# kyutai-labs/pocket-tts

Measured on AMD Instinct MI355X. Metric: audio-seconds/sec (xRT), 100M en model, whole job over all GPUs, higher is better.
Workload: dtype f32

## Files before the change

### pocket_tts_amd/csrc/ptts.hip

```cpp
#include "ptts_host.h"
#include "ptts_flow.h"
#include "ptts_bf16.h"
#include "ptts_lm.h"

#include <algorithm>
#include <array>
#include <cmath>
#include <cstdio>
#include <cstring>

static thread_local std::string g_err;
int fail(int code, const std::string &msg) {
  g_err = msg;
  return code;
}
static thread_local std::string g_launch_err;
bool launch_err_pending() { return !g_launch_err.empty(); }
int take_launch_err() {
  std::string m;
  m.swap(g_launch_err);
  return fail(-4, m);
}
void note_launch_err(const std::string &msg) { if (g_launch_err.empty()) g_launch_err = msg; }

// ... 251 lines not shown
  launch_gemm(st, a, PRE_LNFOLD);
  AttnArgs at;
  at.Q = c.q; at.Kc = c.Kc; at.Vc = c.Vc; at.offset = c.offset; at.H = c.H; at.Tq = c.Tq; at.QB = c.QB;
  at.cap = c.cap; at.ring = c.ring; at.ctx = c.ctx; at.splits = c.splits; at.part = c.part; at.Y = c.ao; at.YF = DF; at.h16 = 0;
  at.pre = c.pre; at.layer = c.layer; at.qlen = c.qlen;
  const int BH = (c.M / c.Tq) * c.H;
  at.nseq = BH / c.H;
  SITE(s3.c_str());
  launch_attention(st, at, BH, c.cascade, -1, c.kv_keys * c.H * 64 * 4 * 2 + 8.0 * c.M * c.D,
                   4.0 * c.kv_keys * c.H * 64 * std::min(c.Tq, 16));
  SITE(s4.c_str());
  a = mk_gemm(T.out, c.ao, DF, c.MT, c.M);
  a.epi = EPI_RES; a.R = c.x_in; a.RF = DF; a.Y = c.x; a.YF = DF; a.ls = T.ls1;
  launch_gemm(st, a, PRE_NONE);
  SITE(s6.c_str());
  a = mk_gemm(T.ff1, c.x, DF, c.MT, c.M);
  a.epi = EPI_STORE; a.act = ACT_GELU; a.Y = c.ff; a.YF = c.FF / 16;
  launch_gemm(st, a, PRE_LNFOLD);
  SITE(s7.c_str());
  a = mk_gemm(T.ff2, c.ff, c.FF / 16, c.MT, c.M);
  a.epi = EPI_RES; a.R = c.x; a.RF = DF; a.Y = c.x_out; a.YF = DF; a.Ydstride = c.out_ds; a.par = c.par; a.ls = T.ls2;
  launch_gemm(st, a, PRE_NONE);
  SITE("");
}

extern "C" int ptts_abi_version(void) { return PTTS_ABI_VERSION; }
extern "C" const char *ptts_last_error(void) { return g_err.c_str(); }

static int seanet_check(const ptts_config &c) {
  if (c.d_model < 64 || c.num_heads < 1 || c.num_layers < 1 || c.m_dim < 64 || c.m_heads < 1 || c.m_layers < 1 || c.ldim < 16 ||
      c.flow_dim < 16 || c.flow_depth < 1 || c.ff_dim < 16 || c.m_ff < 16 || c.n_filters < 1 || c.compress < 1 ||
      c.kernel_size < 1 || c.res_kernel_size < 1 || c.last_kernel_size < 1 || c.ratios[0] < 1 || c.ratios[1] < 1 || c.ratios[2] < 1)
    return fail(-4, "model dimensions must be positive");
  if (c.d_model % 64 || c.d_model / c.num_heads != 64 || c.d_model % c.num_heads) return fail(-4, "FlowLM head dim must be 64");
  if (c.m_dim % c.m_heads || c.m_dim / c.m_heads != 64) return fail(-4, "Mimi head dim must be 64");
  if (c.d_model > 1024 || c.m_dim > 1024 || c.flow_dim > 1024) return fail(-4, "LayerNorm width > 1024 unsupported");
  if (c.ldim % 16 || c.flow_dim % 16 || c.ff_dim % 16 || c.m_ff % 16) return fail(-4, "dims must be multiples of 16");
  if (c.upsample_stride != 16) return fail(-4, "upsample stride must be 16 (one row tile per frame)");
  if ((c.n_filters / c.compress) % 16) return fail(-4, "n_filters/compress must be a multiple of 16");
  return 0;
}

static int build_engine(ptts_engine *e, const ptts_tensor *tensors, int32_t n);
static int build_fp8_codec(ptts_engine *e);
static int sync_host_tables(ptts_engine *e);

static int init_engine_options(ptts_engine *e, int device) {
  e->device = device;
  e->tuner = new Tuner();
  hipDeviceProp_t prop;
  HIPCHK(hipGetDeviceProperties(&prop, device));
  e->n_cus = std::max(1, prop.multiProcessorCount);
  if (const char *v = getenv("PTTS_FLOW_CLUSTER")) e->opt_flow_cluster = atoi(v) != 0;
  if (const char *v = getenv("PTTS_LM_CLUSTER")) e->opt_lm_cluster = atoi(v) != 0;
  if (const char *v = getenv("PTTS_K_ROTATE")) e->opt_k_rotate = atoi(v) != 0;
  if (const char *v = getenv("PTTS_FUSE_RES")) e->opt_fuse_res = atoi(v) != 0;
  if (const char *v = getenv("PTTS_SHARE_PREFIX")) e->opt_share_prefix = atoi(v) != 0;
  if (const char *v = getenv("PTTS_SINGLE_STORE")) e->opt_single_store = atoi(v) != 0;
  if (const char *v = getenv("PTTS_FUSE_PCM")) e->opt_fuse_pcm = atoi(v) != 0;
  if (const char *v = getenv("PTTS_CASCADE")) e->opt_cascade = atoi(v);
  if (const char *v = getenv("PTTS_FLOW_MAX_CUS")) e->opt_flow_max_cus = std::max(8, atoi(v));
  e->opt_flow_max_cus = std::min(e->opt_flow_max_cus, e->n_cus);
  if (const char *v = getenv("PTTS_CODEC_LDS_TARGET")) e->opt_codec_lds_target = std::max(0, std::min(atoi(v), 64 * 1024));
  return 0;
}

extern "C" int ptts_create(const ptts_config *cfg, const ptts_tensor *tensors, int32_t n, int32_t device,
                           ptts_engine **out) {
  return ptts_create_ex(cfg, tensors, n, device, 0, out);
}

extern "C" int ptts_create_ex(const ptts_config *cfg, const ptts_tensor *tensors, int32_t n, int32_t device,
                              int32_t quant_flags, ptts_engine **out) {
  if (!cfg || !tensors || !out) return fail(-1, "null argument");
  if (quant_flags & ~(PTTS_QUANT_ATTENTION | PTTS_QUANT_FFN | PTTS_CODEC_BF16 | PTTS_CODEC_FP8 | PTTS_LM_BF16 | PTTS_CODEC_SPLIT)) return fail(-1, "unknown quantisation group");
  if ((quant_flags & PTTS_CODEC_BF16) && (quant_flags & PTTS_CODEC_FP8)) return fail(-1, "PTTS_CODEC_BF16 and PTTS_CODEC_FP8 are exclusive");
  if ((quant_flags & PTTS_CODEC_SPLIT) && (quant_flags & (PTTS_CODEC_BF16 | PTTS_CODEC_FP8))) return fail(-1, "PTTS_CODEC_SPLIT and the bf16 / fp8 codec are exclusive");
  if ((quant_flags & PTTS_LM_BF16) && (quant_flags & (PTTS_QUANT_ATTENTION | PTTS_QUANT_FFN))) return fail(-1, "PTTS_LM_BF16 and the int8 groups are exclusive");
  CHK(seanet_check(*cfg));
  HIPCHK(hipSetDevice(device));
  ptts_engine *e = new ptts_engine();
  e->cfg = *cfg;
  e->quant_flags = quant_flags;
  int rc = init_engine_options(e, device);
  if (rc == 0) rc = build_engine(e, tensors, n);
  if (rc < 0) {
    const std::string msg = g_err;
    ptts_destroy(e);
    return fail(rc, msg);
  }
  *out = e;
  return 0;
}

static int build_engine(ptts_engine *e, const ptts_tensor *tensors, int32_t n) {
  HIPCHK(hipStreamCreateWithFlags(&e->stream, hipStreamNonBlocking));
  AllocScope alloc_scope(e->stream);
  HIPCHK(hipEventCreate(&e->ev0));
  HIPCHK(hipEventCreate(&e->ev1));
  for (int i = 0; i < n; ++i) e->tmap[tensors[i].name] = &tensors[i];
  const ptts_config &c = e->cfg;
  const int D = c.d_model, FD = c.flow_dim;
  std::string p = "flow_lm.";
  CHK(copy_vec(e, p + "bos_emb", c.ldim, &e->bos));
  CHK(make_freq(e, &e->freq_lm, c.max_period));
  CHK(pack_lin(e, &e->in_linear, {{p + "input_linear.weight", "", D}}, c.ldim, 1));
// ... 867 lines not shown
  if ((int64_t)out.size() + 1 > capacity) return fail(-1, "profile buffer too small");
  memcpy(h_out, out.c_str(), out.size() + 1);
  return (int64_t)out.size();
}


static bool flow_cluster_ok(const ptts_engine *e, const ptts_lm_state *s) {
  const ptts_config &c = e->cfg;
  const int FDF = c.flow_dim / 16, LF = c.ldim / 16;
  if (!e->opt_flow_cluster || c.flow_depth > FLOW_MAX_DEPTH || FDF > 64 || LF > FDF) return false;
  const int kpw = cdiv(std::max(FDF, LF), FLOW_WORKERS);
  if (kpw != 1 && kpw != 2 && kpw != 4) return false;
  if (!e->input_proj.bias || !e->fin.bias) return false;
  for (auto &r : e->res) if (!r.l0.bias || !r.l2.bias) return false;
  return FDF <= std::min(e->opt_flow_max_cus, e->n_cus);
}
static int ensure_flow(ptts_engine *e, ptts_lm_state *s, int steps, hipStream_t st) {
  if (steps <= s->flow_steps) return 0;
  if (s->n_graphs > 0)
    return fail(-1, "lsd_decode_steps grows beyond what this state's captured graphs were built for: destroy the graphs first "
                    "(they hold the old AdaLN / exchange buffers)");
  const ptts_config &c = e->cfg;
  const int FDF = c.flow_dim / 16;
  static const int rt_env = [] { const char *v = getenv("PTTS_FLOW_RT"); return v ? atoi(v) : 1; }();
  s->flow_rt = (rt_env == 2 && s->MT >= 2) ? 2 : 1;
  s->flow_ng = cdiv(s->MT, s->flow_rt);
  HIPCHK(hipStreamSynchronize(st));
  HIPCHK(hipStreamSynchronize(e->stream));
  AllocScope alloc_scope(st);
  hipFree(s->mod); hipFree(s->fexch); hipFree(s->fflags);
  s->mod = nullptr; s->fexch = nullptr; s->fflags = nullptr;
  const size_t rt = (size_t)s->MT * 256;
  const int nph = steps * (2 * c.flow_depth + 2);
  CHK(dallocT(nullptr, &s->mod, (size_t)steps * rt * e->adaln.NT));
  CHK(dallocT(nullptr, &s->fexch, (size_t)s->flow_ng * nph * s->flow_rt * FDF * 256));
  CHK(dallocT(nullptr, &s->fflags, (size_t)s->flow_ng * nph * FDF));
  HIPCHK(hipStreamSynchronize(st));
  s->flow_steps = steps;
  return 0;
}

template <int RT, bool ROWLSD>
static void launch_flow_rt(hipStream_t st, const FlowArgs &fa, int kpw) {
  const dim3 grid(fa.NCL * fa.FDF), block(FLOW_THREADS);
  switch (kpw) {
    case 1: flow_cluster_kernel<RT, 1, ROWLSD><<<grid, block, 0, st>>>(fa); break;
    case 2: flow_cluster_kernel<RT, 2, ROWLSD><<<grid, block, 0, st>>>(fa); break;
    default: flow_cluster_kernel<RT, 4, ROWLSD><<<grid, block, 0, st>>>(fa); break;
  }
}

static int flow_steps_of(const ptts_lm_state *s, int lsd_steps) { return std::max(lsd_steps, s->lsd_cap); }

static void launch_flow_cluster(hipStream_t st, ptts_engine *e, ptts_lm_state *s, int lsd_steps, float *d_latent_out) {
  const ptts_config &c = e->cfg;
  const int FDF = c.flow_dim / 16, LF = c.ldim / 16;
  FlowArgs fa;
  memset(&fa, 0, sizeof fa);
  fa.MT = s->MT; fa.M = s->B; fa.NG = s->flow_ng; fa.NCL = std::max(1, std::min(s->flow_ng, std::min(e->opt_flow_max_cus, e->n_cus) / FDF)); fa.FDF = FDF; fa.LF = LF; fa.AF = e->adaln.NT;
  const bool rowlsd = s->lsd_cap > 0;
  fa.depth = c.flow_depth; fa.steps = rowlsd ? flow_steps_of(s, lsd_steps) : lsd_steps; fa.ldim = c.ldim;
  fa.w_in = e->input_proj.w; fa.b_in = e->input_proj.bias;
  for (int r = 0; r < c.flow_depth; ++r) {
    fa.w_l0[r] = e->res[r].l0.w; fa.b_l0[r] = e->res[r].l0.bias;
    fa.w_l2[r] = e->res[r].l2.w; fa.b_l2[r] = e->res[r].l2.bias;
    fa.ln_w[r] = e->res[r].ln_w; fa.ln_b[r] = e->res[r].ln_b;
  }
  fa.w_fin = e->fin.w; fa.b_fin = e->fin.bias;
  fa.mod = s->mod; fa.mod_step = (long)s->MT * 256 * e->adaln.NT;
  fa.latfm = s->latfm;
  fa.lat = s->lat; fa.lat_out1 = s->lat_prev; fa.lat_out2 = d_latent_out;
  fa.inv_steps = 1.0f / (float)lsd_steps;
  fa.exch = s->fexch; fa.flags = s->fflags; fa.ctr = s->rng_ctr; fa.err = s->ferr;
  fa.row_n = rowlsd ? s->lsd_n : nullptr; fa.row_ndef = lsd_steps;
  const double wbytes = 4.0 * 256 * ((double)FDF * LF + 2.0 * c.flow_depth * FDF * FDF + (double)LF * FDF);
  const double flops = 2.0 * s->B * 256.0 * ((double)FDF * LF + 2.0 * c.flow_depth * FDF * FDF + (double)LF * FDF) * lsd_steps;
  ProfScope ps(st, std::string(rowlsd ? "flow_cluster_rowlsd@" : "flow_cluster@") + std::to_string((long)fa.NCL * FDF * FLOW_THREADS),
               lsd_steps * (wbytes + 4.0 * s->B * 16.0 * e->adaln.NT), flops);
  const int kpw = cdiv(std::max(FDF, LF), FLOW_WORKERS);
  s->coop_wgs = std::max(s->coop_wgs, fa.NCL * FDF);
  if (rowlsd) {
    if (s->flow_rt == 2) launch_flow_rt<2, true>(st, fa, kpw);
    else launch_flow_rt<1, true>(st, fa, kpw);
  } else {
    if (s->flow_rt == 2) launch_flow_rt<2, false>(st, fa, kpw);
    else launch_flow_rt<1, false>(st, fa, kpw);
  }
}


static constexpr int kLmMaxWGs = 256;
static bool lm_cluster_ok(const ptts_engine *e, const ptts_lm_state *s) {
  if (!e->opt_lm_cluster || !e->lm_table) return false;
  if (e->cfg.d_model / 16 > std::min(kLmMaxWGs, e->n_cus)) return false;
  if (s->n_pre > 0) return false;
  return (double)s->kv_plane() * 4.0 < 2.0e9;
}
static int ensure_lm_cluster(ptts_engine *e, ptts_lm_state *s, hipStream_t st) {
  if (s->lexch || !e->lm_table) return 0;
  const ptts_config &c = e->cfg;
  const int DF = c.d_model / 16, FFF = c.ff_dim / 16;
  AllocScope alloc_scope(st);
  CHK(dallocT(nullptr, &s->lexch, (size_t)s->MT * c.num_layers * (4 * DF + FFF) * 256));
  CHK(dallocT(nullptr, &s->lflags, (size_t)s->MT * c.num_layers * 5 * DF));
  HIPCHK(hipStreamSynchronize(st));
  return 0;
}
static void launch_lm_cluster(hipStream_t st, ptts_engine *e, ptts_lm_state *s, Scratch &sc) {
  const ptts_config &c = e->cfg;
  LmArgs la;
  memset(&la, 0, sizeof la);
  la.MT = s->MT; la.M = s->B; la.NG = s->MT; la.DF = c.d_model / 16; la.FFF = c.ff_dim / 16; la.H = c.num_heads;
  la.NCL = std::max(1, std::min(la.NG, std::min(kLmMaxWGs, e->n_cus) / la.DF));
  s->coop_wgs = std::max(s->coop_wgs, la.NCL * la.DF);
  la.L = c.num_layers; la.cap = s->cap;
  la.layers = e->lm_table; la.kv = s->kv; la.kv_plane = (long)s->kv_plane();
  la.offset = s->offset; la.freq = e->freq_lm; la.x = sc.x; la.exch = s->lexch; la.flags = s->lflags;
  la.ctr = s->rng_ctr; la.err = s->ferr; la.ln_eps = 1e-5f;
  double keys = 0;
  for (int b = 0; b < s->B; ++b) keys += s->h_off[b] + 1;
  const double wbytes = 4.0 * 256.0 * c.num_layers * ((double)4 * la.DF * la.DF + 2.0 * la.DF * la.FFF);
  ProfScope ps(st, "lm_cluster@" + std::to_string((long)la.NCL * la.DF * FLOW_THREADS),
               wbytes + c.num_layers * keys * c.num_heads * 64 * 4 * 2,
               c.num_layers * (2.0 * s->B * 256.0 * ((double)4 * la.DF * la.DF + 2.0 * la.DF * la.FFF) + 4.0 * keys * c.num_heads * 64));
  lm_cluster_kernel<0><<<dim3(la.NCL * la.DF), dim3(FLOW_THREADS), 0, st>>>(la);
}

static constexpr int kCoopMaxSlots = 4;
struct CoopSlots { hipEvent_t ev[kCoopMaxSlots] = {}; bool used[kCoopMaxSlots] = {}; unsigned long long next = 0; };
// ... 82 lines not shown
  sc.MT = MT;
  long n4 = (long)MT * (c.d_model / 16) * 64;
  to_fm_kernel<<<cdiv(n4, 256), 256, 0, st>>>(d_emb, sc.x, M, c.d_model, MT);
  lm_layers(st, e, s, sc, M, T);
  add_int_kernel<<<cdiv(s->B, 256), 256, 0, st>>>(s->offset, s->B, T);
  for (auto &o : s->h_off) o += T;
  LAUNCHCHK();
  return 0;
}

extern "C" int ptts_lm_prefill_ragged(ptts_engine *e, ptts_lm_state *s, const float *d_emb, const int32_t *h_len, int32_t t_max,
                                      void *stream) {
  if (!e || !s || !h_len) return fail(-1, "prefill_ragged: null argument");
  ENGINE_LOCK(e);
  if (t_max < 1) return fail(-1, "prefill_ragged: t_max must be >= 1");
  bool any = false;
  for (int b = 0; b < s->B; ++b) {
    if (h_len[b] < 0 || h_len[b] > t_max) return fail(-1, "prefill_ragged: row " + std::to_string(b) + " has length " + std::to_string(h_len[b]) +
                                                              ", expected 0 .. " + std::to_string(t_max));
    any |= h_len[b] > 0;
  }
  for (int b = 0; b < s->B; ++b)
    if (s->h_off[b] + h_len[b] > s->cap) return fail(-5, "prefill: KV cache capacity exceeded");
  if (!any) return 0;
  if (!d_emb) return fail(-1, "prefill_ragged: null argument");
  HIPCHK(hipSetDevice(e->device));
  const ptts_config &c = e->cfg;
  hipStream_t st = S(e, stream);
  const int M = s->B * t_max;
  if (!s->pre.x || s->pre.MT < cdiv(M, 16) || s->pre.QB != cdiv(t_max, 16)) {
    HIPCHK(hipStreamSynchronize(st));
    if (s->pre.x) free_scratch(&s->pre);
    AllocScope alloc_scope(st);
    CHK(alloc_scratch(e, &s->pre, s->B, t_max, c.d_model, c.num_heads, c.ff_dim, s->cap));
  }
  Scratch &sc = s->pre;
  const int MT = cdiv(M, 16);
  sc.MT = MT;
  for (int b0 = 0; b0 < s->B; b0 += 64) {
    IntPack pk;
    const int n = std::min(64, s->B - b0);
    for (int i = 0; i < 64; ++i) pk.v[i] = i < n ? h_len[b0 + i] : 0;
    set_ints_kernel<<<1, 64, 0, st>>>(s->qlen + b0, n, pk);
  }
  long n4 = (long)MT * (c.d_model / 16) * 64;
  to_fm_kernel<<<cdiv(n4, 256), 256, 0, st>>>(d_emb, sc.x, M, c.d_model, MT);
  lm_layers(st, e, s, sc, M, t_max, false, s->qlen, h_len);
  add_rows_kernel<<<cdiv(s->B, 256), 256, 0, st>>>(s->offset, s->qlen, s->B);
  for (int b = 0; b < s->B; ++b) s->h_off[b] += h_len[b];
  LAUNCHCHK();
  return 0;
}

static int coop_wgs_of_step(const ptts_engine *e, const ptts_lm_state *s, int lsd_steps) {
  int w = 0;
  const ptts_config &c = e->cfg;
  if (flow_cluster_ok(e, s) && flow_steps_of(s, lsd_steps) <= s->flow_steps) {
    const int FDF = c.flow_dim / 16;
    w = std::max(1, std::min(s->flow_ng, std::min(e->opt_flow_max_cus, e->n_cus) / FDF)) * FDF;
  }
  if (lm_cluster_ok(e, s) && s->lexch) {
    const int DF = c.d_model / 16;
    w = std::max(w, std::max(1, std::min(s->MT, std::min(kLmMaxWGs, e->n_cus) / DF)) * DF);
  }
  return w;
}

static int lm_step_enqueue(hipStream_t st, ptts_engine *e, ptts_lm_state *s, const float *d_latent_in,
                           const float *d_noise, int lsd_steps, float eos_thr, float *d_latent_out,
                           float *d_eos_logit, uint8_t *d_is_eos) {
  const ptts_config &c = e->cfg;
  bind_engine(e);
  const int B = s->B, MT = s->MT, D = c.d_model, FD = c.flow_dim, DF = D / 16, FDF = FD / 16, LF = c.ldim / 16;
  Scratch &sc = s->dec;
  s->coop_wgs = 0;
  const float *tcomb = e->tcomb[lsd_steps];
  SITE("lm.prep");
  if (e->in_linear.w && !e->in_linear.bias && e->in_linear.KF == LF) {
    ProfScope ps(st, "prep_in", 16.0 * B * c.ldim + 4.0 * (D * c.ldim + B * D), 2.0 * B * D * c.ldim);
    const int nb_gemm = cdiv(DF * MT, 4), nb_prep = cdiv(MT * LF * 64, 256);
    prep_in_kernel<<<nb_gemm + nb_prep + cdiv(B * 32, 256), 256, 0, st>>>(
        d_latent_in ? d_latent_in : s->lat_prev, e->bos, d_noise, e->in_linear.w, sc.x, s->lat, s->latfm, B, c.ldim, MT, DF, s->rng_std,
        s->rng_seed, s->rng_ctr, s->rsamp(), nb_gemm, nb_prep, RopeArgs{s->offset, e->freq_lm, sc.rope, B, 1});
  } else {
    {
      ProfScope ps(st, "prep_lm", 16.0 * B * c.ldim, 0);
      const int nb_prep = cdiv(MT * LF * 64, 256);
      prep_lm_kernel<<<nb_prep + cdiv(B * 32, 256), 256, 0, st>>>(d_latent_in ? d_latent_in : s->lat_prev, e->bos, d_noise,
                                                                   s->xlat, s->lat, s->latfm, B, c.ldim, MT, s->rng_std,
                                                                   s->rng_seed, s->rng_ctr, s->rsamp(), nb_prep,
                                                                   RopeArgs{s->offset, e->freq_lm, sc.rope, B, 1});
    }
    SITE("lm.in_linear");
    GemmArgs a0 = mk_gemm(e->in_linear, s->xlat, LF, MT, B);
    a0.Y = sc.x; a0.YF = DF;
    launch_gemm(st, a0, PRE_NONE);
  }
  GemmArgs a;
  if (lm_cluster_ok(e, s) && s->lexch) {
    SITE("lm.cluster");
    launch_lm_cluster(st, e, s, sc);
  } else {
    lm_layers(st, e, s, sc, B, 1, true);
  }
  SITE("flow.head");
  a = mk_gemm(e->head, sc.x, DF, MT, B);
  a.epi = EPI_HEAD; a.Y = s->ce; a.YF = FDF; a.head_nt = FDF; a.eos_thr = eos_thr;
  a.eos_on = s->samp_on; a.eos_row = s->samp_eos;
  a.eos_logit = s->eos_logit; a.is_eos = s->is_eos;
  a.eos_logit2 = d_eos_logit; a.is_eos2 = d_is_eos;
  a.tail_offset = s->offset; a.tail_ctr = s->rng_ctr; a.tail_rctr = s->seed_ctr; a.tail_active = s->active;
  const bool silu_in_head = lsd_steps == 1 && s->lsd_cap == 0;
  if (silu_in_head) { a.act = ACT_SILU; a.prevec = tcomb; }
  launch_gemm(st, a, PRE_LNFOLD);
  const int AF = e->adaln.NT;
  const bool rowlsd = s->lsd_cap > 0;
  const int nit = rowlsd ? flow_steps_of(s, lsd_steps) : lsd_steps;
  auto row_lsd = [&](GemmArgs &g, int i) {
    g.row_n = s->lsd_n; g.row_tab = s->lsd_tab; g.row_ndef = lsd_steps; g.row_i = i;
  };
  if (flow_cluster_ok(e, s) && nit <= s->flow_steps) {
    if (rowlsd) {
      SITE("flow.adaln");
      a = mk_gemm(e->adaln, s->ce, FDF, MT, B);
      a.prevec = tcomb; a.Y = s->mod; a.YF = AF;
      row_lsd(a, 0);
      a.row_nz = nit; a.row_zstride = (long)MT * 256 * AF;
      launch_gemm(st, a, PRE_ADDSILU_ROW);
    } else {
      for (int i = 0; i < lsd_steps; ++i) {
        SITE("flow.adaln");
        a = mk_gemm(e->adaln, s->ce, FDF, MT, B);
        a.prevec = tcomb + (size_t)i * FD; a.Y = s->mod + (size_t)i * MT * 256 * AF; a.YF = AF;
        launch_gemm(st, a, silu_in_head ? PRE_NONE : PRE_ADDSILU);
      }
    }
    SITE("flow.cluster");
    launch_flow_cluster(st, e, s, lsd_steps, d_latent_out);
    s->latfm_noise = true;
  } else {
  s->latfm_noise = false;
  for (int i = 0; i < nit; ++i) {
    SITE("flow.adaln");
    a = mk_gemm(e->adaln, s->ce, FDF, MT, B);
    a.prevec = tcomb + (size_t)i * FD; a.Y = s->mod; a.YF = AF;
    if (rowlsd) {
      a.prevec = tcomb;
      row_lsd(a, i);
      launch_gemm(st, a, PRE_ADDSILU_ROW);
    } else {
      launch_gemm(st, a, silu_in_head ? PRE_NONE : PRE_ADDSILU);
    }
    SITE("flow.input_proj");
    a = mk_gemm(e->input_proj, s->latfm, LF, MT, B);
    a.Y = s->fx; a.YF = FDF;
    a.stat_out = s->fstat;
    launch_gemm(st, a, PRE_NONE);
    for (int r = 0; r < c.flow_depth; ++r) {
      const float *shift = s->mod + (size_t)(r * 3 * FDF) * 256;
      const float *scale = shift + (size_t)FDF * 256;
      const float *gate = scale + (size_t)FDF * 256;
      SITE("flow.res.l0");
      a = mk_gemm(e->res[r].l0, s->fx, FDF, MT, B);
      a.act = ACT_SILU; a.Y = s->f1; a.YF = FDF;
      a.lnm_w = e->res[r].ln_w; a.lnm_b = e->res[r].ln_b; a.mod_shift = shift; a.mod_scale = scale; a.modF = AF;
      a.ln_eps = 1e-6f;
      a.stat_in = s->fstat; a.stat_nt = FDF;
      launch_gemm(st, a, PRE_LNMOD);
      SITE("flow.res.l2");
      a = mk_gemm(e->res[r].l2, s->f1, FDF, MT, B);
      a.epi = EPI_GATE; a.R = s->fx; a.RF = FDF; a.G = gate; a.GF = AF; a.Y = s->fx; a.YF = FDF;
      a.stat_out = s->fstat;
      launch_gemm(st, a, PRE_NONE);
    }
    const float *shift = s->mod + (size_t)(c.flow_depth * 3 * FDF) * 256;
    const float *scale = shift + (size_t)FDF * 256;
    SITE("flow.final");
    a = mk_gemm(e->fin, s->fx, FDF, MT, B);
    a.lnm_w = nullptr; a.lnm_b = nullptr; a.mod_shift = shift; a.mod_scale = scale; a.modF = AF; a.ln_eps = 1e-6f;
    a.stat_in = s->fstat; a.stat_nt = FDF;
    a.epi = EPI_LATENT; a.lat = s->lat; a.ldim = c.ldim; a.inv_steps = 1.0f / (float)lsd_steps; a.Y = s->latfm; a.YF = LF;
    if (i == lsd_steps - 1) { a.lat_out1 = s->lat_prev; a.lat_out2 = d_latent_out; }
    if (rowlsd) {
      row_lsd(a, i);
      a.lat_out1 = s->lat_prev; a.lat_out2 = d_latent_out;
    }
    launch_gemm(st, a, rowlsd ? PRE_LNMOD_ROW : PRE_LNMOD);
  }
  }
  SITE("");
  return 0;
// ... 820 lines not shown
    if (hipEventRecord(join, side) != hipSuccess) return fail(-2, "join record");
    if (hipStreamWaitEvent(st, join, 0) != hipSuccess) return fail(-2, "join wait");
    return 0;
  });
  hipEventDestroy(fork);
  hipEventDestroy(join);
  hipStreamDestroy(side);
  if (rc < 0) { g->lm = nullptr; g->mimi = nullptr; ptts_graph_destroy(g); return rc; }
  g->coop_wgs = s->coop_wgs;
  s->n_graphs += 1;
  *out = g;
  return 0;
}

extern "C" int ptts_graph_launch(ptts_graph *g, void *stream) {
  ptts_engine *e = g->lm ? g->lm->e : g->mimi->e;
  ENGINE_LOCK(e);
  HIPCHK(hipSetDevice(e->device));
  if (g->lm) {
    for (int b = 0; b < g->lm->B; ++b)
      if (g->lm->h_off[b] + 1 > g->lm->cap) return fail(-5, "decode: KV cache capacity exceeded");
  }
  {
    if (g->coop_wgs > 0 && g->cu_checked != S(e, stream)) {
      if (g->coop_wgs > stream_cu_count(S(e, stream), e->n_cus))
        return fail(-1, "graph launch: the stream's CU mask is smaller than the cooperative launch captured in this graph");
      g->cu_checked = S(e, stream);
    }
    CoopGuard guard(e->device, S(e, stream), g->coop_wgs, e->n_cus);
    HIPCHK(hipGraphLaunch(g->exec_c && g->lm && g->lm->n_pre > 0 ? g->exec_c : g->exec, S(e, stream)));
    if (guard.finish() < 0) return fail(-2, "graph launch: could not chain the cooperative launch behind its predecessor");
  }
  if (g->lm) for (int b = 0; b < g->lm->B; ++b) g->lm->h_off[b] += g->lm->h_active[b];
  if (g->mimi) g->mimi->h_frame += 1;
  return 0;
}

extern "C" void ptts_graph_destroy(ptts_graph *g) {
  if (!g) return;
  if (g->lm && g->exec && g->lm->n_graphs > 0) g->lm->n_graphs -= 1;
  if (g->exec) hipGraphExecDestroy(g->exec);
  if (g->graph) hipGraphDestroy(g->graph);
  if (g->exec_c) hipGraphExecDestroy(g->exec_c);
  if (g->graph_c) hipGraphDestroy(g->graph_c);
  if (g->cap_stream) hipStreamDestroy(g->cap_stream);
  delete g;
}

extern "C" int ptts_set_option(ptts_engine *e, const char *key, int32_t value) {
  if (!e || !key) return fail(-1, "null argument");
  ENGINE_LOCK(e);
  const std::string k(key);
  if (k == "flow_cluster") e->opt_flow_cluster = value != 0;
  else if (k == "lm_cluster") e->opt_lm_cluster = value != 0;
  else if (k == "k_rotate") e->opt_k_rotate = value != 0;
  else if (k == "fuse_res") e->opt_fuse_res = value != 0;
  else if (k == "share_prefix") e->opt_share_prefix = value != 0;
  else if (k == "single_store") e->opt_single_store = value != 0;
  else if (k == "fuse_pcm") e->opt_fuse_pcm = value != 0;
  else if (k == "debug_taps") e->opt_debug_taps = value != 0;
  else if (k == "prefix_cascade") e->opt_cascade = value == 1 ? 423 : value;
  else if (k == "codec_lds_target") {
    if (value < 0 || value > 64 * 1024) return fail(-1, "codec_lds_target must be in [0, 65536]");
    e->opt_codec_lds_target = value;
  }
  else if (k == "flow_max_cus") {
    if (value < 8 || value > e->n_cus) return fail(-1, "flow_max_cus must be in [8, CUs of the device = " + std::to_string(e->n_cus) + "]");
    e->opt_flow_max_cus = value;
  }
  else return fail(-1, "unknown option " + k);
  return 0;
}
extern "C" int ptts_lm_state_error(ptts_lm_state *s, void *stream) {
  if (!s) return fail(-1, "null state");
  int h = 0;
  hipStream_t st = S(s->e, stream);
  HIPCHK(hipSetDevice(s->e->device));
  HIPCHK(hipMemcpyAsync(&h, s->ferr, sizeof(int), hipMemcpyDeviceToHost, st));
  HIPCHK(hipMemsetAsync(s->ferr, 0, sizeof(int), st));
  HIPCHK(hipStreamSynchronize(st));
  return h != 0;
}
extern "C" int ptts_debug_set_error(ptts_lm_state *s, int32_t value, void *stream) {
  if (!s) return fail(-1, "null state");
  hipStream_t st = S(s->e, stream);
  HIPCHK(hipSetDevice(s->e->device));
  HIPCHK(hipMemsetAsync(s->ferr, value ? 1 : 0, 1, st));
  HIPCHK(hipStreamSynchronize(st));
  return 0;
}
extern "C" int ptts_stream_create_masked(ptts_engine *e, int32_t cu_lo, int32_t cu_hi, void **out) {
  if (!e || !out) return fail(-1, "bad argument");
  HIPCHK(hipSetDevice(e->device));
  hipDeviceProp_t prop;
  HIPCHK(hipGetDeviceProperties(&prop, e->device));
  const int ncu = prop.multiProcessorCount, nxcd = 8, per = ncu / nxcd, words = (ncu + 31) / 32;
  if (cu_lo < 0 || cu_hi > per || cu_lo >= cu_hi) return fail(-1, "CU range must lie inside [0, CUs per XCD)");
  std::vector<uint32_t> mask(words, 0u);
  for (int i = 0; i < ncu; ++i) {
    const int c = i / nxcd;
    if (c >= cu_lo && c < cu_hi) mask[i >> 5] |= 1u << (i & 31);
  }
  hipStream_t st = nullptr;
  HIPCHK(hipExtStreamCreateWithCUMask(&st, (uint32_t)words, mask.data()));
  *out = (void *)st;
  return 0;
// ... 70 lines not shown
```

### pocket_tts_amd/csrc/ptts_flow.h

```cpp
#pragma once
#include "ptts_kernels.h"

#define FLOW_MAX_DEPTH 12
#define FLOW_WORKERS 8
#define FLOW_THREADS (64 * (FLOW_WORKERS + 1))
#define FLOW_SPIN_LIMIT 400000u

typedef unsigned u32x4 __attribute__((ext_vector_type(4)));
typedef unsigned long long u64;

struct FlowArgs {
  int MT, M, NG, NCL, FDF, LF, AF, depth, steps, ldim;
  const float *w_in, *b_in;
  const float *w_l0[FLOW_MAX_DEPTH], *b_l0[FLOW_MAX_DEPTH], *w_l2[FLOW_MAX_DEPTH], *b_l2[FLOW_MAX_DEPTH];
  const float *ln_w[FLOW_MAX_DEPTH], *ln_b[FLOW_MAX_DEPTH];
  const float *w_fin, *b_fin;
  const float *mod;
  long mod_step;
  const float *latfm;
  float *lat, *lat_out1, *lat_out2;
  float inv_steps;
  float *exch;
  u64 *flags;
  const int *ctr;
  int *err;
  const int *row_n;
  int row_ndef;
};

__device__ __forceinline__ __amdgpu_buffer_rsrc_t flow_rsrc(const void *p) {
  return __builtin_amdgcn_make_buffer_rsrc(const_cast<void *>(p), 0, 0x7ffffff0, 0x00020000);
}
__device__ __forceinline__ f32x4 flow_ld_sc1(__amdgpu_buffer_rsrc_t r, unsigned byte_off) {
  return __builtin_bit_cast(f32x4, __builtin_amdgcn_raw_buffer_load_b128(r, (int)byte_off, 0, 16));
}
__device__ __forceinline__ void flow_st_sc1(__amdgpu_buffer_rsrc_t r, unsigned byte_off, f32x4 v) {
  __builtin_amdgcn_raw_buffer_store_b128(__builtin_bit_cast(u32x4, v), r, (int)byte_off, 0, 16);
}

__device__ __forceinline__ bool flow_wait(const u64 *f, int np, u64 epoch, int lane, int *err) {
  for (unsigned spins = 0;; ++spins) {
    const u64 v = lane < np ? __hip_atomic_load(f + lane, __ATOMIC_RELAXED, __HIP_MEMORY_SCOPE_AGENT) : epoch;
    if (__all(v == epoch)) return true;
    if (spins > FLOW_SPIN_LIMIT) {
      if (lane == 0) atomicExch(err, 1);
      return false;
    }
    __builtin_amdgcn_s_sleep(2);
  }
}

template <int RT, int KPW, bool ROWLSD = false>
__global__ __launch_bounds__(FLOW_THREADS) void flow_cluster_kernel(FlowArgs a) {
  const int lane = threadIdx.x & 63, wave = threadIdx.x >> 6;
  const int FDF = a.FDF, LF = a.LF;
  const int cl = blockIdx.x / a.FDF, j = blockIdx.x % a.FDF;
  const bool coord = wave == FLOW_WORKERS;
  const int PPS = 2 * a.depth + 2, NPH = a.steps * PPS;
  __shared__ f32x4 red[FLOW_WORKERS][RT][64];
  __shared__ float st[FLOW_WORKERS][RT][16][2];
  const u64 ebase = ((u64)(unsigned)(*a.ctr) + 1ull) << 16;
  const f32x4 zero4 = {0.f, 0.f, 0.f, 0.f};
  bool dead = false;
  for (int grp = cl; grp < a.NG; grp += a.NCL) {
  const int mt0 = grp * RT;
  float *ex = a.exch + (size_t)grp * NPH * RT * FDF * 256;
  u64 *fl = a.flags + (size_t)grp * NPH * FDF;
  const __amdgpu_buffer_rsrc_t rs = flow_rsrc(ex);
  __syncthreads();

  int mtc[RT];
#pragma unroll
  for (int t = 0; t < RT; ++t) mtc[t] = min(mt0 + t, a.MT - 1);
  int nph = NPH;
  int nrow[RT];
  if constexpr (ROWLSD) {
    int mx = 0;
    const int mg = 16 * mt0 + lane;
    if (lane < RT * 16 && mg < a.M) mx = row_lsd_n(a.row_n, a.row_ndef, mg);
#pragma unroll
    for (int o = 32; o; o >>= 1) mx = max(mx, __shfl_xor(mx, o));
    nph = __builtin_amdgcn_readfirstlane(mx) * PPS;
#pragma unroll
    for (int t = 0; t < RT; ++t) {
      const int m = 16 * (mt0 + t) + (lane & 15);
      nrow[t] = m < a.M ? row_lsd_n(a.row_n, a.row_ndef, m) : 1;
    }
  }

  auto kind_of = [&](int ph) { return ph == 0 ? 0 : ph == PPS - 1 ? 3 : 1 + ((ph - 1) & 1); };
  auto wtile = [&](int ph, int &KF, bool &use) -> const float * {
    const int k = kind_of(ph), r = (ph - 1) >> 1;
    use = true;
    if (k == 0) { KF = LF; return a.w_in + (size_t)j * LF * 256; }
    KF = FDF;
    if (k == 1) return a.w_l0[r] + (size_t)j * FDF * 256;
    if (k == 2) return a.w_l2[r] + (size_t)j * FDF * 256;
    use = j < LF;
    return a.w_fin + (size_t)(use ? j : 0) * FDF * 256;
  };
  auto bias_of = [&](int ph) -> const float * {
    const int k = kind_of(ph), r = (ph - 1) >> 1;
    return (k == 0 ? a.b_in : k == 1 ? a.b_l0[r] : k == 2 ? a.b_l2[r] : a.b_fin) + (k == 3 && j >= LF ? 0 : 16 * j) + 4 * (lane >> 4);
  };

  f32x4 w[KPW];
  auto load_w = [&](int ph) {
    int KF;
    bool use;
    const float *Wt = wtile(ph, KF, use);
#pragma unroll
    for (int u = 0; u < KPW; ++u) {
      const int kf = wave * KPW + u;
      const f32x4 v = *(const f32x4 *)(Wt + (size_t)min(kf, KF - 1) * 256 + lane * 4);
      w[u] = (use && kf < KF) ? v : zero4;
    }
  };
  f32x4 xres[RT], latv[RT], e_bias = zero4, e_gate[RT], n_bias = zero4, n_gate[RT];
#pragma unroll
  for (int t = 0; t < RT; ++t) xres[t] = latv[t] = e_gate[t] = n_gate[t] = zero4;
  auto load_epi = [&](int p, f32x4 &bias, f32x4 *gate) {
    const int i = p / PPS, ph = p - i * PPS;
    bias = *(const f32x4 *)bias_of(ph);
    if (kind_of(ph) == 2) {
      const int r = (ph - 1) >> 1;
#pragma unroll
      for (int t = 0; t < RT; ++t)
        gate[t] = *(const f32x4 *)(a.mod + (size_t)i * a.mod_step + (((size_t)mtc[t] * a.AF + r * 3 * FDF + 2 * FDF + j) * 64 + lane) * 4);
    }
  };
  if (coord) {
    load_epi(0, e_bias, e_gate);
    if (j < LF) {
#pragma unroll
      for (int t = 0; t < RT; ++t) latv[t] = *(const f32x4 *)(a.latfm + (((size_t)mtc[t] * LF + j) * 64 + lane) * 4);
    }
  } else {
    load_w(0);
  }

  for (int p = 0; p < nph; ++p) {
    const int i = p / PPS, ph = p - i * PPS;
    const int kind = kind_of(ph);
    const int KF = kind == 0 ? LF : FDF;
    const bool lnmod = kind == 1 || kind == 3;
    if (coord && p > 0 && !dead) {
      const int np = ph == 0 ? LF : FDF;
      if (!flow_wait(fl + (size_t)(p - 1) * FDF, np, ebase | (u64)p, lane, a.err)) dead = true;
    }
    __syncthreads();
    f32x4 x[RT][KPW], ma[RT][KPW], mb[RT][KPW];
    const int r = (ph - 1) >> 1;
    if (!coord) {
      if (p == 0) {
#pragma unroll
        for (int t = 0; t < RT; ++t)
#pragma unroll
          for (int u = 0; u < KPW; ++u) {
            const int kf = wave * KPW + u;
            const f32x4 v = *(const f32x4 *)(a.latfm + (((size_t)mtc[t] * LF + min(kf, KF - 1)) * 64 + lane) * 4);
            x[t][u] = kf < KF ? v : zero4;
          }
      } else {
        const unsigned sbase = (unsigned)(p - 1) * RT * FDF * 1024u;
#pragma unroll
        for (int t = 0; t < RT; ++t)
#pragma unroll
          for (int u = 0; u < KPW; ++u) {
            const int kf = wave * KPW + u;
            const f32x4 v = flow_ld_sc1(rs, sbase + ((unsigned)(t * FDF + min(kf, KF - 1)) * 64u + lane) * 16u);
            x[t][u] = kf < KF ? v : zero4;
          }
      }
      if (lnmod) {
        const float *mbase = a.mod + (size_t)i * a.mod_step;
        const int sh0 = kind == 1 ? r * 3 * FDF : a.depth * 3 * FDF;
#pragma unroll
        for (int u = 0; u < KPW; ++u) {
          const int kf = min(wave * KPW + u, KF - 1);
          f32x4 lw = {1.f, 1.f, 1.f, 1.f}, lb = zero4;
          if (kind == 1) {
            lw = *(const f32x4 *)(a.ln_w[r] + 16 * kf + 4 * (lane >> 4));
            lb = *(const f32x4 *)(a.ln_b[r] + 16 * kf + 4 * (lane >> 4));
          }
#pragma unroll
          for (int t = 0; t < RT; ++t) {
            const float *mp = mbase + (((size_t)mtc[t] * a.AF + sh0 + kf) * 64 + lane) * 4;
            const f32x4 shv = *(const f32x4 *)mp, scv = 1.0f + *(const f32x4 *)(mp + (size_t)FDF * 256);
            ma[t][u] = lw * scv;
            mb[t][u] = lb * scv + shv;
          }
        }
#pragma unroll
        for (int t = 0; t < RT; ++t) {
          float s1 = 0.f, s2 = 0.f;
#pragma unroll
          for (int u = 0; u < KPW; ++u) {
            const f32x4 v = x[t][u];
            s1 += (v.x + v.y) + (v.z + v.w);
// ... 87 lines not shown
```

### pocket_tts_amd/csrc/ptts_host.h

```cpp
#pragma once
#include "ptts_kernels.h"
#include "ptts_ext.h"

#include <array>
#include <map>
#include <mutex>
#include <string>
#include <vector>

#include "../../include/ptts.h"

#pragma GCC visibility push(hidden)

int fail(int code, const std::string &msg);
#define HIPCHK(x)                                                                                      \
  do {                                                                                                 \
    hipError_t e_ = (x);                                                                               \
    if (e_ != hipSuccess)                                                                              \
      return fail(-2, std::string(#x) + ": " + hipGetErrorString(e_) + " @" + std::to_string(__LINE__)); \
  } while (0)
#define CHK(x)            \
  do {                    \
    int r_ = (x);         \
    if (r_ < 0) return r_; \
// ... 43 lines not shown
struct Tuner {
  std::map<TuneKey, int> table;
  bool active = false;
  void *flush = nullptr;
  size_t flush_bytes = 0;
  hipEvent_t e0 = nullptr, e1 = nullptr;
  std::string log;
};
struct LmLayerP;
struct ptts_engine {
  ptts_config cfg;
  int device = 0;
  hipStream_t stream = nullptr;
  hipEvent_t ev0 = nullptr, ev1 = nullptr;
  std::vector<void *> allocs;
  std::map<void *, size_t> alloc_bytes;
  size_t n_build_allocs = 0;
  const ptts_tensor *blob_dummy = nullptr;
  int blob_has_encoder = 0;
  std::map<std::string, const ptts_tensor *> tmap;
  float *bos = nullptr, *freq_lm = nullptr;
  Lin in_linear;
  std::vector<TrLayer> lm;
  float *outnorm_w, *outnorm_b;
  Lin head, adaln, input_proj, fin;
  struct Res { float *ln_w, *ln_b; Lin l0, l2; };
  std::vector<Res> res;
  Lin te_l0[2], te_l2[2];
  float *te_freqs[2], *te_alpha[2];
  std::map<int, float *> tcomb;
  std::map<int, float *> tpack;
  float *te_scratch = nullptr;
  float *emb_std, *emb_mean, *up_w, *freq_mimi;
  float *quant_w = nullptr;
  std::vector<TrLayer> mm;
  Lin conv0, convtr[3], res_a[3], res_b[3], conv_last;
  float *conv_last_w = nullptr, *conv_last_b = nullptr;
  bool codec_bf16 = false;
  int64_t mimi_bytes_h = 0;
  bool codec_split = false;
  bool codec_fp8 = false;
  float *d_f8s = nullptr;
  float f8s[16] = {};
  int64_t mimi_bytes_f8 = 0;
  int ring = 0;
  bool has_encoder = false;
  Lin enc_conv0, enc_res_a[3], enc_res_b[3], enc_down[3], enc_final, enc_downsample, speaker_proj;
  std::vector<TrLayer> enc_tr;
  float *zeros = nullptr;
  int64_t lm_bytes = 0, mimi_bytes = 0;
  Tuner *tuner = nullptr;
  Profiler prof;
  int opt_flow_cluster = 1;
  int opt_lm_cluster = 0;
  LmLayerP *lm_table = nullptr;
  int opt_k_rotate = 0;
  long fuse_res_min_rows = 0;
  int opt_codec_lds_target = 56 * 1024;
  int opt_fuse_pcm = 1;
  int opt_debug_taps = 0;
  int opt_single_store = 1;
  int opt_fuse_res = 1;
  int opt_flow_max_cus = 128;
  int opt_share_prefix = 1;
  int opt_cascade = 423;
  int n_cus = 256;
  std::recursive_mutex mu;
  int quant_flags = 0;
};
#define ENGINE_LOCK(e) std::lock_guard<std::recursive_mutex> lock_((e)->mu)

struct Scratch {
  float *x = nullptr, *h = nullptr, *ao = nullptr, *ff = nullptr, *q = nullptr, *part = nullptr, *rope = nullptr;
  int MT = 0, QB = 0, splits_cap = 0;
};

struct ptts_lm_state {
  ptts_engine *e;
  int B, cap, MT;
  float *kv = nullptr;
  int *offset = nullptr;
  int *qlen = nullptr;
  std::vector<int> h_off;
  Scratch dec, pre;
  float *xlat, *c, *ce, *mod, *latfm, *fx, *fh, *f1;
  float *fstat = nullptr;
  float *fexch = nullptr;
  unsigned long long *fflags = nullptr;
  int *ferr = nullptr;
  int flow_steps = 0, flow_rt = 1, flow_ng = 1;
  int lsd_cap = 0;
  const float *lsd_tab = nullptr;
  int *lsd_n = nullptr;
  KvPrefix *d_pre = nullptr;
  std::vector<KvPrefix> h_pre;
  std::vector<ptts_lm_state *> pre_owner;
  int casc_mode = -1;
  int n_pre = 0;
  int borrowers = 0;
  bool zombie = false;
  int n_graphs = 0;
  int coop_wgs = 0;
  float *lexch = nullptr;
  unsigned long long *lflags = nullptr;
  float *lat, *lat_prev;
  float *eos_logit;
// ... 104 lines not shown
```

### pocket_tts_amd/csrc/ptts_kernels.h

```cpp
#pragma once
#include <hip/hip_runtime.h>
#include <stdint.h>
#include <type_traits>

typedef float f32x4 __attribute__((ext_vector_type(4)));
typedef int i32x4 __attribute__((ext_vector_type(4)));

typedef __bf16 bf16x8 __attribute__((ext_vector_type(8)));
typedef __bf16 bf16x4 __attribute__((ext_vector_type(4)));
__device__ __forceinline__ bf16x4 to_bf16x4(f32x4 v) { return __builtin_convertvector(v, bf16x4); }
__device__ __forceinline__ f32x4 from_bf16x4(bf16x4 v) { return __builtin_convertvector(v, f32x4); }
__device__ __forceinline__ size_t fmh_off(size_t row, int n0, int KB) {
  return (((row >> 4) * KB + (n0 >> 5)) * 64 + (((n0 & 31) >> 3) * 16 + (row & 15))) * 8 + (n0 & 7);
}

__device__ __forceinline__ unsigned to_f8x4(f32x4 v) {
  v.x = fminf(fmaxf(v.x, -448.f), 448.f); v.y = fminf(fmaxf(v.y, -448.f), 448.f);
  v.z = fminf(fmaxf(v.z, -448.f), 448.f); v.w = fminf(fmaxf(v.w, -448.f), 448.f);
  int r = __builtin_amdgcn_cvt_pk_fp8_f32(v.x, v.y, 0, false);
  r = __builtin_amdgcn_cvt_pk_fp8_f32(v.z, v.w, r, true);
  return (unsigned)r;
}

#ifndef PTTS_ABLATE
// ... 1218 lines not shown
  return z;
}

struct RopeArgs {
  const int *offset;
  const float *freq;
  float *tab;
  int M, Tq;
};
__device__ __forceinline__ void rope_table_entry(const RopeArgs &r, int i) {
  if (i >= r.M * 32) return;
  int m = i >> 5, f = i & 31;
  int b = m / r.Tq, t = m - b * r.Tq;
  float sn, cs;
  sincosf(r.freq[f] * (float)(r.offset[b] + t), &sn, &cs);
  r.tab[2 * i] = cs;
  r.tab[2 * i + 1] = sn;
}

static __global__ void prep_lm_kernel(const float *lat_in, const float *bos, const float *noise, float *x_fm, float *lat,
                               float *lat_fm, int B, int ldim, int MT, float rng_std, unsigned long long rng_seed,
                               const int *rng_ctr, RowSampling rsamp, int nb_prep, RopeArgs rope) {
  if ((int)blockIdx.x >= nb_prep) {
    rope_table_entry(rope, (blockIdx.x - nb_prep) * blockDim.x + threadIdx.x);
    return;
  }
  int i = blockIdx.x * blockDim.x + threadIdx.x;
  int KF = ldim / 16;
  if (i >= MT * KF * 64) return;
  int lane = i & 63;
  int f = i >> 6;
  int kf = f % KF, mt = f / KF;
  int m = 16 * mt + (lane & 15);
  int k = 16 * kf + 4 * (lane >> 4);
  f32x4 v = (f32x4){0.f, 0.f, 0.f, 0.f}, z = v;
  if (m < B) {
    v = *(const f32x4 *)(lat_in + (size_t)m * ldim + k);
    f32x4 b = *(const f32x4 *)(bos + k);
    v.x = v.x != v.x ? b.x : v.x;
    v.y = v.y != v.y ? b.y : v.y;
    v.z = v.z != v.z ? b.z : v.z;
    v.w = v.w != v.w ? b.w : v.w;
    if (noise) {
      z = *(const f32x4 *)(noise + (size_t)m * ldim + k);
    } else {
      z = device_noise(rsamp, m, k, ldim, rng_std, rng_seed, rng_ctr);
    }
  }
  *(f32x4 *)(x_fm + (size_t)i * 4) = v;
  *(f32x4 *)(lat_fm + (size_t)i * 4) = z;
  if (m < B) *(f32x4 *)(lat + (size_t)m * ldim + k) = z;
}

static __global__ __launch_bounds__(256) void prep_in_kernel(const float *lat_in, const float *bos, const float *noise, const float *w_in,
                                                             float *x_out, float *lat, float *lat_fm, int B, int ldim, int MT, int DF,
                                                             float rng_std, unsigned long long rng_seed, const int *rng_ctr,
                                                             RowSampling rsamp, int nb_gemm, int nb_prep, RopeArgs rope) {
  const int LF = ldim / 16;
  if ((int)blockIdx.x < nb_gemm) {
    const int lane = threadIdx.x & 63, tile = blockIdx.x * 4 + (threadIdx.x >> 6);
    if (tile >= DF * MT) return;
    const int nt = tile % DF, mt = tile / DF;
    const int m = 16 * mt + (lane & 15), g = lane >> 4;
    f32x4 acc = {0.f, 0.f, 0.f, 0.f};
    for (int kf = 0; kf < LF; ++kf) {
      const int k = 16 * kf + 4 * g;
      f32x4 v = {0.f, 0.f, 0.f, 0.f};
      if (m < B) {
        v = *(const f32x4 *)(lat_in + (size_t)m * ldim + k);
        const f32x4 b = *(const f32x4 *)(bos + k);
        v.x = v.x != v.x ? b.x : v.x; v.y = v.y != v.y ? b.y : v.y; v.z = v.z != v.z ? b.z : v.z; v.w = v.w != v.w ? b.w : v.w;
      }
      const f32x4 w = *(const f32x4 *)(w_in + (((size_t)nt * LF + kf) * 64 + lane) * 4);
#pragma unroll
      for (int c = 0; c < 4; ++c) acc = __builtin_amdgcn_mfma_f32_16x16x4f32(w[c], v[c], acc, 0, 0, 0);
    }
    *(f32x4 *)(x_out + (((size_t)mt * DF + nt) * 64 + lane) * 4) = acc;
    return;
  }
  if ((int)blockIdx.x >= nb_gemm + nb_prep) {
    rope_table_entry(rope, (blockIdx.x - nb_gemm - nb_prep) * blockDim.x + threadIdx.x);
    return;
  }
  const int i = (blockIdx.x - nb_gemm) * blockDim.x + threadIdx.x;
  if (i >= MT * LF * 64) return;
  const int lane = i & 63, f = i >> 6;
  const int kf = f % LF, mt = f / LF;
  const int m = 16 * mt + (lane & 15), k = 16 * kf + 4 * (lane >> 4);
  f32x4 z = {0.f, 0.f, 0.f, 0.f};
  if (m < B) {
    if (noise) {
      z = *(const f32x4 *)(noise + (size_t)m * ldim + k);
    } else {
      z = device_noise(rsamp, m, k, ldim, rng_std, rng_seed, rng_ctr);
    }
  }
  *(f32x4 *)(lat_fm + (size_t)i * 4) = z;
  if (m < B) *(f32x4 *)(lat + (size_t)m * ldim + k) = z;
}

static __global__ void mimi_prologue_kernel(const float *lat, const float *std, const float *mean, const float *wq,
                                     const float *wup, float *zq, long zdstride, const int *par_p, float *out, int B,
                                     int ldim, int C, int s, int nb_main, RopeArgs rope, int h16) {
  if ((int)blockIdx.x >= nb_main) {
    rope_table_entry(rope, (blockIdx.x - nb_main) * blockDim.x + threadIdx.x);
    return;
  }
  const int C4 = C / 4, CF = C / 16;
  const long i = (long)blockIdx.x * blockDim.x + threadIdx.x;
  if (i >= (long)B * C4 * s) return;
  const int t = (int)(i % s);
  const int c = (int)((i / s) % C4) * 4, b = (int)(i / ((long)s * C4));
  const int par = *par_p & 1;
  f32x4 zc = {0.f, 0.f, 0.f, 0.f};
  const float *lr = lat + (size_t)b * ldim;
  for (int k = 0; k < ldim; k += 4) {
    const f32x4 z = *(const f32x4 *)(lr + k) * *(const f32x4 *)(std + k) + *(const f32x4 *)(mean + k);
    const f32x4 w0 = *(const f32x4 *)(wq + (size_t)(c + 0) * ldim + k), w1 = *(const f32x4 *)(wq + (size_t)(c + 1) * ldim + k);
    const f32x4 w2 = *(const f32x4 *)(wq + (size_t)(c + 2) * ldim + k), w3 = *(const f32x4 *)(wq + (size_t)(c + 3) * ldim + k);
    zc.x += (z.x * w0.x + z.y * w0.y) + (z.z * w0.z + z.w * w0.w);
    zc.y += (z.x * w1.x + z.y * w1.y) + (z.z * w1.z + z.w * w1.w);
    zc.z += (z.x * w2.x + z.y * w2.y) + (z.z * w2.z + z.w * w2.w);
    zc.w += (z.x * w3.x + z.y * w3.y) + (z.z * w3.z + z.w * w3.w);
  }
  const size_t zi = (((size_t)(b >> 4) * CF + (c >> 4)) * 64 + 16 * ((c & 15) >> 2) + (b & 15)) * 4;
  const f32x4 zp = *(const f32x4 *)(zq + (par ^ 1) * zdstride + zi);
  if (t == 0) *(f32x4 *)(zq + par * zdstride + zi) = zc;
  const int k2 = 2 * s;
  f32x4 o;
  o.x = zc.x * wup[(c + 0) * k2 + t] + zp.x * wup[(c + 0) * k2 + s + t];
  o.y = zc.y * wup[(c + 1) * k2 + t] + zp.y * wup[(c + 1) * k2 + s + t];
  o.z = zc.z * wup[(c + 2) * k2 + t] + zp.z * wup[(c + 2) * k2 + s + t];
  o.w = zc.w * wup[(c + 3) * k2 + t] + zp.w * wup[(c + 3) * k2 + s + t];
  const long m = (long)b * s + t;
  if (h16) *(bf16x4 *)((__bf16 *)out + fmh_off((size_t)m, c, C / 32)) = to_bf16x4(o);
  else *(f32x4 *)(out + (((size_t)(m >> 4) * CF + (c >> 4)) * 64 + 16 * ((c & 15) >> 2) + (m & 15)) * 4) = o;
}
// ... 866 lines not shown
```

Before: 5934.

## Fold flow input projection into prep kernel to skip first flow phase

When LSD uses a single step, the flow network's input projection (noise latent times input_proj weights plus bias) is now computed inside the prep_in kernel, right where the noise is generated. The result is written directly into the flow cluster's exchange buffer, and the cooperative flow kernel starts at phase 1. This removes one serialized phase, with its inter-workgroup wait, from the persistent flow kernel. The cost is extra MFMA blocks in prep_in, and correctness depends on matching the exchange layout and the KPW partial-sum order.

```diff
diff --git a/pocket_tts_amd/csrc/ptts.hip b/pocket_tts_amd/csrc/ptts.hip
--- a/pocket_tts_amd/csrc/ptts.hip
+++ b/pocket_tts_amd/csrc/ptts.hip
@@ -327,6 +327,7 @@
   HIPCHK(hipGetDeviceProperties(&prop, device));
   e->n_cus = std::max(1, prop.multiProcessorCount);
   if (const char *v = getenv("PTTS_FLOW_CLUSTER")) e->opt_flow_cluster = atoi(v) != 0;
+  if (const char *v = getenv("PTTS_FLOW_FOLD")) e->opt_flow_fold = atoi(v) != 0;
   if (const char *v = getenv("PTTS_LM_CLUSTER")) e->opt_lm_cluster = atoi(v) != 0;
   if (const char *v = getenv("PTTS_K_ROTATE")) e->opt_k_rotate = atoi(v) != 0;
   if (const char *v = getenv("PTTS_FUSE_RES")) e->opt_fuse_res = atoi(v) != 0;
@@ -1300,7 +1301,7 @@
 
 static int flow_steps_of(const ptts_lm_state *s, int lsd_steps) { return std::max(lsd_steps, s->lsd_cap); }
 
-static void launch_flow_cluster(hipStream_t st, ptts_engine *e, ptts_lm_state *s, int lsd_steps, float *d_latent_out) {
+static void launch_flow_cluster(hipStream_t st, ptts_engine *e, ptts_lm_state *s, int lsd_steps, float *d_latent_out, bool fold) {
   const ptts_config &c = e->cfg;
   const int FDF = c.flow_dim / 16, LF = c.ldim / 16;
   FlowArgs fa;
@@ -1321,8 +1322,10 @@
   fa.inv_steps = 1.0f / (float)lsd_steps;
   fa.exch = s->fexch; fa.flags = s->fflags; fa.ctr = s->rng_ctr; fa.err = s->ferr;
   fa.row_n = rowlsd ? s->lsd_n : nullptr; fa.row_ndef = lsd_steps;
-  const double wbytes = 4.0 * 256 * ((double)FDF * LF + 2.0 * c.flow_depth * FDF * FDF + (double)LF * FDF);
-  const double flops = 2.0 * s->B * 256.0 * ((double)FDF * LF + 2.0 * c.flow_depth * FDF * FDF + (double)LF * FDF) * lsd_steps;
+  fa.p0 = fold ? 1 : 0;
+  const double tiles = (fold ? 0.0 : (double)FDF * LF) + 2.0 * c.flow_depth * FDF * FDF + (double)LF * FDF;
+  const double wbytes = 4.0 * 256 * tiles;
+  const double flops = 2.0 * s->B * 256.0 * tiles * lsd_steps;
   ProfScope ps(st, std::string(rowlsd ? "flow_cluster_rowlsd@" : "flow_cluster@") + std::to_string((long)fa.NCL * FDF * FLOW_THREADS),
                lsd_steps * (wbytes + 4.0 * s->B * 16.0 * e->adaln.NT), flops);
   const int kpw = cdiv(std::max(FDF, LF), FLOW_WORKERS);
@@ -1511,6 +1514,13 @@
   return 0;
 }
 
+static bool flow_fold_ok(const ptts_engine *e, const ptts_lm_state *s, int lsd_steps) {
+  if (!e->opt_flow_fold || lsd_steps != 1 || s->lsd_cap != 0) return false;
+  if (!flow_cluster_ok(e, s) || s->flow_steps < 1 || !s->fexch) return false;
+  if (e->cfg.ldim / 16 > PREP_FOLD_MAXLF) return false;
+  return e->input_proj.w && !e->input_proj.wq && !e->input_proj.wb16;
+}
+
 static int coop_wgs_of_step(const ptts_engine *e, const ptts_lm_state *s, int lsd_steps) {
   int w = 0;
   const ptts_config &c = e->cfg;
@@ -1534,13 +1544,23 @@
   Scratch &sc = s->dec;
   s->coop_wgs = 0;
   const float *tcomb = e->tcomb[lsd_steps];
+  bool fold = false;
   SITE("lm.prep");
   if (e->in_linear.w && !e->in_linear.bias && e->in_linear.KF == LF) {
-    ProfScope ps(st, "prep_in", 16.0 * B * c.ldim + 4.0 * (D * c.ldim + B * D), 2.0 * B * D * c.ldim);
-    const int nb_gemm = cdiv(DF * MT, 4), nb_prep = cdiv(MT * LF * 64, 256);
-    prep_in_kernel<<<nb_gemm + nb_prep + cdiv(B * 32, 256), 256, 0, st>>>(
+    fold = flow_fold_ok(e, s, lsd_steps);
+    ProfScope ps(st, "prep_in", 16.0 * B * c.ldim + 4.0 * (D * c.ldim + B * D) + (fold ? 4.0 * (FD * c.ldim + B * FD) : 0.0),
+                 2.0 * B * (D + (fold ? FD : 0)) * c.ldim);
+    const int nb_gemm = cdiv(DF * MT, 4), nb_prep = fold ? 0 : cdiv(MT * LF * 64, 256), nb_rope = cdiv(B * 32, 256);
+    PrepFold pf = {};
+    if (fold) {
+      pf.w = e->input_proj.w; pf.bias = e->input_proj.bias; pf.exch = s->fexch;
+      pf.gstride = (long)(2 * c.flow_depth + 2) * s->flow_rt * FDF * 256;
+      pf.FDF = FDF; pf.RT = s->flow_rt; pf.nb = MT * cdiv(FDF, 4);
+      pf.KPW = cdiv(std::max(FDF, LF), FLOW_WORKERS);
+    }
+    prep_in_kernel<<<pf.nb + nb_gemm + nb_prep + nb_rope, 256, 0, st>>>(
         d_latent_in ? d_latent_in : s->lat_prev, e->bos, d_noise, e->in_linear.w, sc.x, s->lat, s->latfm, B, c.ldim, MT, DF, s->rng_std,
-        s->rng_seed, s->rng_ctr, s->rsamp(), nb_gemm, nb_prep, RopeArgs{s->offset, e->freq_lm, sc.rope, B, 1});
+        s->rng_seed, s->rng_ctr, s->rsamp(), nb_gemm, nb_prep, RopeArgs{s->offset, e->freq_lm, sc.rope, B, 1}, pf);
   } else {
     {
       ProfScope ps(st, "prep_lm", 16.0 * B * c.ldim, 0);
@@ -1595,7 +1615,7 @@
       }
     }
     SITE("flow.cluster");
-    launch_flow_cluster(st, e, s, lsd_steps, d_latent_out);
+    launch_flow_cluster(st, e, s, lsd_steps, d_latent_out, fold);
     s->latfm_noise = true;
   } else {
   s->latfm_noise = false;
@@ -2522,6 +2542,7 @@
   ENGINE_LOCK(e);
   const std::string k(key);
   if (k == "flow_cluster") e->opt_flow_cluster = value != 0;
+  else if (k == "flow_fold") e->opt_flow_fold = value != 0;
   else if (k == "lm_cluster") e->opt_lm_cluster = value != 0;
   else if (k == "k_rotate") e->opt_k_rotate = value != 0;
   else if (k == "fuse_res") e->opt_fuse_res = value != 0;
diff --git a/pocket_tts_amd/csrc/ptts_flow.h b/pocket_tts_amd/csrc/ptts_flow.h
--- a/pocket_tts_amd/csrc/ptts_flow.h
+++ b/pocket_tts_amd/csrc/ptts_flow.h
@@ -26,6 +26,7 @@
   int *err;
   const int *row_n;
   int row_ndef;
+  int p0;
 };
 
 __device__ __forceinline__ __amdgpu_buffer_rsrc_t flow_rsrc(const void *p) {
@@ -130,21 +131,25 @@
     }
   };
   if (coord) {
-    load_epi(0, e_bias, e_gate);
+    load_epi(a.p0, e_bias, e_gate);
+    if (a.p0) {
+#pragma unroll
+      for (int t = 0; t < RT; ++t) xres[t] = flow_ld_sc1(rs, ((unsigned)(t * FDF + j) * 64u + lane) * 16u);
+    }
     if (j < LF) {
 #pragma unroll
       for (int t = 0; t < RT; ++t) latv[t] = *(const f32x4 *)(a.latfm + (((size_t)mtc[t] * LF + j) * 64 + lane) * 4);
     }
   } else {
-    load_w(0);
-  }
-
-  for (int p = 0; p < nph; ++p) {
+    load_w(a.p0);
+  }
+
+  for (int p = a.p0; p < nph; ++p) {
     const int i = p / PPS, ph = p - i * PPS;
     const int kind = kind_of(ph);
     const int KF = kind == 0 ? LF : FDF;
     const bool lnmod = kind == 1 || kind == 3;
-    if (coord && p > 0 && !dead) {
+    if (coord && p > a.p0 && !dead) {
       const int np = ph == 0 ? LF : FDF;
       if (!flow_wait(fl + (size_t)(p - 1) * FDF, np, ebase | (u64)p, lane, a.err)) dead = true;
     }
diff --git a/pocket_tts_amd/csrc/ptts_host.h b/pocket_tts_amd/csrc/ptts_host.h
--- a/pocket_tts_amd/csrc/ptts_host.h
+++ b/pocket_tts_amd/csrc/ptts_host.h
@@ -119,6 +119,7 @@
   Tuner *tuner = nullptr;
   Profiler prof;
   int opt_flow_cluster = 1;
+  int opt_flow_fold = 1;
   int opt_lm_cluster = 0;
   LmLayerP *lm_table = nullptr;
   int opt_k_rotate = 0;
diff --git a/pocket_tts_amd/csrc/ptts_kernels.h b/pocket_tts_amd/csrc/ptts_kernels.h
--- a/pocket_tts_amd/csrc/ptts_kernels.h
+++ b/pocket_tts_amd/csrc/ptts_kernels.h
@@ -1294,13 +1294,65 @@
   if (m < B) *(f32x4 *)(lat + (size_t)m * ldim + k) = z;
 }
 
+#define PREP_FOLD_MAXLF 4
+struct PrepFold {
+  const float *w, *bias;
+  float *exch;
+  long gstride;
+  int FDF, RT, nb;
+  int KPW;
+};
 static __global__ __launch_bounds__(256) void prep_in_kernel(const float *lat_in, const float *bos, const float *noise, const float *w_in,
                                                              float *x_out, float *lat, float *lat_fm, int B, int ldim, int MT, int DF,
                                                              float rng_std, unsigned long long rng_seed, const int *rng_ctr,
-                                                             RowSampling rsamp, int nb_gemm, int nb_prep, RopeArgs rope) {
+                                                             RowSampling rsamp, int nb_gemm, int nb_prep, RopeArgs rope,
+                                                             PrepFold fold) {
   const int LF = ldim / 16;
-  if ((int)blockIdx.x < nb_gemm) {
-    const int lane = threadIdx.x & 63, tile = blockIdx.x * 4 + (threadIdx.x >> 6);
+  if ((int)blockIdx.x < fold.nb) {
+    __shared__ f32x4 zs[PREP_FOLD_MAXLF][64];
+    const int lane = threadIdx.x & 63, wave = threadIdx.x >> 6;
+    const int NTG = (fold.FDF + 3) >> 2, bid = blockIdx.x;
+    const int mt = bid / NTG, ntg = bid - mt * NTG, nt = 4 * ntg + wave;
+    const int m = 16 * mt + (lane & 15), g = lane >> 4;
+    const bool mine = nt < fold.FDF;
+    f32x4 w[PREP_FOLD_MAXLF], bias = {0.f, 0.f, 0.f, 0.f};
+#pragma unroll
+    for (int kf = 0; kf < PREP_FOLD_MAXLF; ++kf)
+      if (mine && kf < LF) w[kf] = *(const f32x4 *)(fold.w + (((size_t)nt * LF + kf) * 64 + lane) * 4);
+    if (mine) bias = *(const f32x4 *)(fold.bias + 16 * nt + 4 * g);
+    for (int kf = wave; kf < LF; kf += 4) {
+      const int k = 16 * kf + 4 * g;
+      f32x4 z = {0.f, 0.f, 0.f, 0.f};
+      if (m < B) z = noise ? *(const f32x4 *)(noise + (size_t)m * ldim + k) : device_noise(rsamp, m, k, ldim, rng_std, rng_seed, rng_ctr);
+      zs[kf][lane] = z;
+      if (ntg == 0) {
+        *(f32x4 *)(lat_fm + (((size_t)mt * LF + kf) * 64 + lane) * 4) = z;
+        if (m < B) *(f32x4 *)(lat + (size_t)m * ldim + k) = z;
+      }
+    }
+    __syncthreads();
+    if (!mine) return;
+    f32x4 acc = {0.f, 0.f, 0.f, 0.f}, part = acc;
+#pragma unroll
+    for (int kf = 0; kf < PREP_FOLD_MAXLF; ++kf) {
+      if (kf < LF) {
+        const f32x4 z = zs[kf][lane];
+#pragma unroll
+        for (int c = 0; c < 4; ++c) part = __builtin_amdgcn_mfma_f32_16x16x4f32(w[kf][c], z[c], part, 0, 0, 0);
+        if ((kf + 1) % fold.KPW == 0 || kf + 1 == LF) {
+          acc = kf < fold.KPW ? part : acc + part;
+          part = (f32x4){0.f, 0.f, 0.f, 0.f};
+        }
+      }
+    }
+    acc += bias;
+    const int grp = mt / fold.RT, t = mt - grp * fold.RT;
+    *(f32x4 *)(fold.exch + (size_t)grp * fold.gstride + (((size_t)t * fold.FDF + nt) * 64 + lane) * 4) = acc;
+    return;
+  }
+  const int bx = blockIdx.x - fold.nb;
+  if (bx < nb_gemm) {
+    const int lane = threadIdx.x & 63, tile = bx * 4 + (threadIdx.x >> 6);
     if (tile >= DF * MT) return;
     const int nt = tile % DF, mt = tile / DF;
     const int m = 16 * mt + (lane & 15), g = lane >> 4;
@@ -1320,11 +1372,11 @@
     *(f32x4 *)(x_out + (((size_t)mt * DF + nt) * 64 + lane) * 4) = acc;
     return;
   }
-  if ((int)blockIdx.x >= nb_gemm + nb_prep) {
-    rope_table_entry(rope, (blockIdx.x - nb_gemm - nb_prep) * blockDim.x + threadIdx.x);
+  if (bx >= nb_gemm + nb_prep) {
+    rope_table_entry(rope, (bx - nb_gemm - nb_prep) * blockDim.x + threadIdx.x);
     return;
   }
-  const int i = (blockIdx.x - nb_gemm) * blockDim.x + threadIdx.x;
+  const int i = (bx - nb_gemm) * blockDim.x + threadIdx.x;
   if (i >= MT * LF * 64) return;
   const int lane = i & 63, f = i >> 6;
   const int kf = f % LF, mt = f / LF;
```

New measurement: 5923. Within noise of the previous version (-0.2%).
